# YannDubs/disentangling-vae

Measured on NVIDIA H100. Metric: images/sec, higher is better.
Workload: dtype f32

## Files before the change

disentangling-vae_b200/csrc/dv_conv_tc.cu:

```cuda
#include "dv_common.cuh"
#include "dv_ptx.cuh"

namespace dv {
namespace tc {

using namespace ptx;

constexpr int kATile = 128 * 128;
constexpr int kBTap = 64 * 128;
constexpr int kBBytes = kTaps * kBTap;
constexpr int kConsumers = 8;
constexpr int kThreads = (kConsumers + 1) * 32;
constexpr int kSmemMax = 232448;

__device__ __forceinline__ void consumers_sync() { asm volatile("bar.sync 1, %0;" ::"n"(kConsumers * 32) : "memory"); }

__device__ __forceinline__ void fold_tap(float (&tot)[16], float (&acc)[16]) {
  fence_regs(acc);
#pragma unroll
  for (int i = 0; i < 16; ++i) tot[i] += acc[i];
}

__device__ __forceinline__ void product(float (&acc)[16], float (&acc_prev)[16], float (&corr)[16], float (&tot)[16],
                                        uint32_t (&ah)[16], uint32_t (&al)[16], uint32_t a_base, int p0, int p1,
                                        uint32_t keep0, uint32_t keep1, int t, uint32_t tap_base, int corr_accumulate) {
#pragma unroll
  for (int ks = 0; ks < 4; ++ks) {
    wgmma_wait<3>();
    if (ks == 3) fold_tap(tot, acc_prev);
    split_tf32(lds32(a_base + swz128(p0, 8 * ks + t)) & keep0, ah[4 * ks + 0], al[4 * ks + 0]);
    split_tf32(lds32(a_base + swz128(p1, 8 * ks + t)) & keep1, ah[4 * ks + 1], al[4 * ks + 1]);
    split_tf32(lds32(a_base + swz128(p0, 8 * ks + t + 4)) & keep0, ah[4 * ks + 2], al[4 * ks + 2]);
    split_tf32(lds32(a_base + swz128(p1, 8 * ks + t + 4)) & keep1, ah[4 * ks + 3], al[4 * ks + 3]);
    fence_regs(acc);
    fence_regs(corr);
    wgmma_fence();
    const uint64_t w_hi = wgmma_desc_k128(tap_base + 32 * ks), w_lo = wgmma_desc_k128(tap_base + 32 * 128 + 32 * ks);
    wgmma_m64n32k8_rs(acc, ah + 4 * ks, w_hi, ks);
    wgmma_m64n32k8_rs(corr, ah + 4 * ks, w_lo, ks | corr_accumulate);
    wgmma_m64n32k8_rs(corr, al + 4 * ks, w_hi, 1);
    wgmma_commit();
  }
}

struct DownGeom {
  int B, H, W;
  int rows_per_tile;
  int num_tiles;
  long long total_px;
};
constexpr int kDownStages = 5;
struct DownBarriers {
  uint64_t raw_full[kDownStages], raw_empty[kDownStages];
  uint64_t b_full;
  float bias[32];
  float csum[kConsumers][32];
};
constexpr int kDownSmem = kBBytes + kDownStages * kATile + 1024 + 2048;
static_assert(sizeof(DownBarriers) <= 2048, "barrier block too large");
static_assert(kDownSmem <= kSmemMax, "smem");

__global__ void __launch_bounds__(kThreads, 1)
conv_down32_mma_kernel(const __grid_constant__ CUtensorMap tmap_a, const __grid_constant__ CUtensorMap tmap_b,
                       const float* __restrict__ bias, const float* __restrict__ mask, float* __restrict__ lo,
                       DownGeom g, int act, float* __restrict__ colsum_part,
                       const uint32_t* __restrict__ mask_bits, uint32_t* __restrict__ bits_out) {
  extern __shared__ uint8_t smem_raw[];
  uint8_t* smem = align1024(smem_raw);
  uint8_t* Bs = smem;
  uint8_t* Raw = smem + kBBytes;
  DownBarriers* bars = reinterpret_cast<DownBarriers*>(Raw + kDownStages * kATile);
  const int warp = threadIdx.x >> 5, lane = threadIdx.x & 31;
  if (threadIdx.x == 0) {
    for (int s = 0; s < kDownStages; ++s) { mbar_init(&bars->raw_full[s], 1); mbar_init(&bars->raw_empty[s], kConsumers); }
    mbar_init(&bars->b_full, 1);
    fence_mbar_init();
  }
  if (threadIdx.x < 32) bars->bias[threadIdx.x] = bias ? bias[threadIdx.x] : 0.f;
  __syncthreads();

  if (warp == kConsumers) {
    if (lane != 0) return;
    prefetch_tmap(&tmap_a); prefetch_tmap(&tmap_b);
    mbar_arrive_expect_tx(&bars->b_full, kBBytes);
    for (int tap = 0; tap < kTaps; ++tap) tma_load_2d(Bs + tap * kBTap, &tmap_b, &bars->b_full, 0, tap * 64);
    int stage = 0; uint32_t phase = 0;
    for (int tile = blockIdx.x; tile < g.num_tiles; tile += gridDim.x) {
      const int r0 = tile * g.rows_per_tile;
      const int b0 = r0 / g.H, i0 = r0 % g.H;
      if (tile + (int)gridDim.x < g.num_tiles) {
        const int rn = (tile + gridDim.x) * g.rows_per_tile;
        const int bn = rn / g.H, in_ = rn % g.H;
        for (int t4 = 0; t4 < 4; ++t4) tma_prefetch_4d(&tmap_a, 0, (t4 & 1), 2 * in_ + (t4 >> 1), bn);
      }
      for (int tap = 0; tap < kTaps; ++tap) {
        const int kh = tap >> 2, kw = tap & 3;
        mbar_wait(&bars->raw_empty[stage], phase ^ 1);
        mbar_arrive_expect_tx(&bars->raw_full[stage], kATile);
        tma_load_4d(Raw + stage * kATile, &tmap_a, &bars->raw_full[stage], 0, kw - 1, 2 * i0 - 1 + kh, b0);
        if (++stage == kDownStages) { stage = 0; phase ^= 1; }
      }
    }
    return;
  }

  const int gq = lane >> 2, t = lane & 3;
  const int r0 = warp * 16 + gq;
  const uint32_t bs = smem_u32(Bs), raw0 = smem_u32(Raw);
  float csum[4][2] = {};
  mbar_wait(&bars->b_full, 0);
  int stage = 0; uint32_t phase = 0;
  uint32_t ah[16], al[16];
  auto tap_product = [&](float (&acc)[16], float (&acc_prev)[16], float (&corr)[16], float (&tot)[16], int tap) {
    mbar_wait(&bars->raw_full[stage], phase);
    product(acc, acc_prev, corr, tot, ah, al, raw0 + stage * kATile, r0, r0 + 8, ~0u, ~0u, t, bs + tap * kBTap, tap);
    __syncwarp();
    if (lane == 0) mbar_arrive(&bars->raw_empty[stage]);
    if (++stage == kDownStages) { stage = 0; phase ^= 1; }
  };
  for (int tile = blockIdx.x; tile < g.num_tiles; tile += gridDim.x) {
    float tot[16] = {}, corr[16], acc[2][16];
#pragma unroll
    for (int i = 0; i < 16; ++i) acc[1][i] = 0.f;
#pragma unroll 1
    for (int tap = 0; tap < kTaps; tap += 2) {
      tap_product(acc[0], acc[1], corr, tot, tap);
      tap_product(acc[1], acc[0], corr, tot, tap + 1);
    }
    wgmma_wait<0>();
    fold_tap(tot, acc[1]);
    fence_regs(corr);
#pragma unroll
    for (int h = 0; h < 2; ++h) {
      const long long p = (long long)tile * 128 + r0 + 8 * h;
      const bool valid = p < g.total_px;
      uint32_t mb = 0xffffffffu;
      if (mask_bits && valid) mb = __ldg(mask_bits + p);
      const float* mk = (mask && !mask_bits && valid) ? mask + p * 32 : nullptr;
      uint32_t ob = 0u;
#pragma unroll
      for (int nt = 0; nt < 4; ++nt) {
        const int c = nt * 8 + 2 * t;
        float v[2];
#pragma unroll
        for (int e = 0; e < 2; ++e) {
          float x = (tot[4 * nt + 2 * h + e] + corr[4 * nt + 2 * h + e]) + bars->bias[c + e];
          if (act == DV_ACT_RELU) x = fmaxf(x, 0.f);
          v[e] = ((mb >> (c + e)) & 1u) ? x : 0.f;
        }
        if (mk) {
          const float2 m2 = __ldg(reinterpret_cast<const float2*>(mk + c));
          v[0] = m2.x > 0.f ? v[0] : 0.f; v[1] = m2.y > 0.f ? v[1] : 0.f;
        }
        if (valid) *reinterpret_cast<float2*>(lo + p * 32 + c) = make_float2(v[0], v[1]);
        else v[0] = v[1] = 0.f;
        ob |= (v[0] > 0.f ? 1u : 0u) << c | (v[1] > 0.f ? 1u : 0u) << (c + 1);
        csum[nt][0] += v[0]; csum[nt][1] += v[1];
      }
      ob |= __shfl_xor_sync(0xffffffffu, ob, 1);
      ob |= __shfl_xor_sync(0xffffffffu, ob, 2);
      if (bits_out && valid && t == 0) bits_out[p] = ob;
    }
  }
  if (colsum_part) {
#pragma unroll
    for (int nt = 0; nt < 4; ++nt)
#pragma unroll
      for (int e = 0; e < 2; ++e) {
        float s = csum[nt][e];
        s += __shfl_xor_sync(0xffffffffu, s, 4);
        s += __shfl_xor_sync(0xffffffffu, s, 8);
        s += __shfl_xor_sync(0xffffffffu, s, 16);
        if (gq == 0) bars->csum[warp][nt * 8 + 2 * t + e] = s;
      }
    consumers_sync();
    if (warp == 0) {
      float s = 0.f;
      for (int w = 0; w < kConsumers; ++w) s += bars->csum[w][lane];
      colsum_part[blockIdx.x * 32 + lane] = s;
    }
  }
}

constexpr int kWtSlots = kConsumers;
struct WtBarriers {
  uint64_t raw_full[kWtSlots], raw_empty[kWtSlots];
  uint64_t l_full[2], l_empty[2];
  float lsum[kConsumers][32];
};
constexpr int kWtTotFloats = 2 * 32 * 32;
constexpr int kWtSmem = kWtSlots * kATile + 2 * kATile + 2048 + kConsumers * kWtTotFloats * 4 + 1024;
static_assert(sizeof(WtBarriers) <= 2048, "barrier block too large");
static_assert(kWtSmem <= kSmemMax, "smem");

struct WtGeom {
  int B, H, W, rows_per_tile, num_tiles, tiles_per_cta;
};

__global__ void __launch_bounds__(kThreads, 1)
conv_wgrad32_mma_kernel(const __grid_constant__ CUtensorMap tmap_hi, const __grid_constant__ CUtensorMap tmap_lo,
                        float* __restrict__ ws, WtGeom g) {
  extern __shared__ uint8_t smem_raw[];
  uint8_t* smem = align1024(smem_raw);
  uint8_t* Raw = smem;
  uint8_t* Ls = smem + kWtSlots * kATile;
  WtBarriers* bars = reinterpret_cast<WtBarriers*>(Ls + 2 * kATile);
  const int warp = threadIdx.x >> 5, lane = threadIdx.x & 31;
  float* tot = reinterpret_cast<float*>(Ls + 2 * kATile + 2048) + warp * kWtTotFloats + lane;
  const int t_begin = blockIdx.x * g.tiles_per_cta;
  const int t_end = min(g.num_tiles, t_begin + g.tiles_per_cta);

  if (threadIdx.x == 0) {
    for (int s = 0; s < kWtSlots; ++s) { mbar_init(&bars->raw_full[s], 1); mbar_init(&bars->raw_empty[s], 1); }
    for (int s = 0; s < 2; ++s) { mbar_init(&bars->l_full[s], 1); mbar_init(&bars->l_empty[s], kConsumers); }
    fence_mbar_init();
  }
  __syncthreads();

  if (warp == kConsumers) {
    if (lane != 0) return;
    prefetch_tmap(&tmap_hi); prefetch_tmap(&tmap_lo);
    uint32_t tseq = 0;
    for (int tile = t_begin; tile < t_end; ++tile, ++tseq) {
      const int r0 = tile * g.rows_per_tile;
      const int b0 = r0 / g.H, i0 = r0 % g.H;
      if (tile + 1 < t_end) {
        const int rn = (tile + 1) * g.rows_per_tile;
        const int bn = rn / g.H, in_ = rn % g.H;
        for (int t4 = 0; t4 < 4; ++t4) tma_prefetch_4d(&tmap_hi, 0, (t4 & 1), 2 * in_ + (t4 >> 1), bn);
        tma_prefetch_4d(&tmap_lo, 0, 0, in_, bn);
      }
      const int lb = tseq & 1;
      mbar_wait(&bars->l_empty[lb], ((tseq >> 1) & 1u) ^ 1u);
      mbar_arrive_expect_tx(&bars->l_full[lb], kATile);
      tma_load_4d(Ls + lb * kATile, &tmap_lo, &bars->l_full[lb], 0, 0, i0, b0);
      for (int tap = 0; tap < kTaps; ++tap) {
        const int kh = tap >> 2, kw = tap & 3, slot = tap & 7;
        const uint32_t use = tseq * 2 + (tap >> 3);
        mbar_wait(&bars->raw_empty[slot], (use & 1u) ^ 1u);
        mbar_arrive_expect_tx(&bars->raw_full[slot], kATile);
        tma_load_4d(Raw + slot * kATile, &tmap_hi, &bars->raw_full[slot], 0, kw - 1, 2 * i0 - 1 + kh, b0);
      }
    }
    return;
  }

  const int gq = lane >> 2, t = lane & 3;
  const uint32_t slot_base = smem_u32(Raw) + warp * kATile, l0 = smem_u32(Ls);
  for (int k = 0; k < 64; ++k) tot[k * 32] = 0.f;
  float lsum = 0.f;
  uint32_t tseq = 0;
  for (int tile = t_begin; tile < t_end; ++tile, ++tseq) {
    const int lb = tseq & 1;
    mbar_wait(&bars->l_full[lb], (tseq >> 1) & 1u);
    const uint32_t l_base = l0 + lb * kATile;
#pragma unroll 4
    for (int r = 0; r < 16; ++r) lsum += __uint_as_float(lds32(l_base + swz128(warp * 16 + r, lane)));
#pragma unroll 1
    for (int j = 0; j < 2; ++j) {
      const uint32_t use = tseq * 2 + j;
      mbar_wait(&bars->raw_full[warp], use & 1u);
      float mn[2][4][4] = {}, cr[2][4][4] = {};
#pragma unroll 1
      for (int ks = 0; ks < 16; ++ks) {
        const int px0 = 8 * ks + 2 * t, px1 = px0 + 1;
        uint32_t ah[2][4], al[2][4], bh[4][2], bl[4][2];
#pragma unroll
        for (int mt = 0; mt < 2; ++mt) {
          const int c = mt * 16 + gq;
          uint32_t a[4];
          a[0] = lds32(slot_base + swz128(px0, c));
          a[1] = lds32(slot_base + swz128(px0, c + 8));
          a[2] = lds32(slot_base + swz128(px1, c));
          a[3] = lds32(slot_base + swz128(px1, c + 8));
#pragma unroll
          for (int e = 0; e < 4; ++e) split_tf32(a[e], ah[mt][e], al[mt][e]);
        }
#pragma unroll
        for (int nt = 0; nt < 4; ++nt) {
          const int cl = nt * 8 + gq;
          split_tf32(lds32(l_base + swz128(px0, cl)), bh[nt][0], bl[nt][0]);
          split_tf32(lds32(l_base + swz128(px1, cl)), bh[nt][1], bl[nt][1]);
        }
#pragma unroll
        for (int mt = 0; mt < 2; ++mt)
#pragma unroll
          for (int nt = 0; nt < 4; ++nt) mma_3xtf32(mn[mt][nt], cr[mt][nt], ah[mt], al[mt], bh[nt], bl[nt]);
      }
      __syncwarp();
      if (lane == 0) mbar_arrive(&bars->raw_empty[warp]);
#pragma unroll
      for (int mt = 0; mt < 2; ++mt)
#pragma unroll
        for (int nt = 0; nt < 4; ++nt)
#pragma unroll
          for (int e = 0; e < 4; ++e) tot[(j * 32 + (mt * 4 + nt) * 4 + e) * 32] += mn[mt][nt][e] + cr[mt][nt][e];
    }
    __syncwarp();
    if (lane == 0) mbar_arrive(&bars->l_empty[lb]);
  }

  float* out = ws + (long long)blockIdx.x * (kTaps * 32 + 1) * kLoCh;
#pragma unroll
  for (int j = 0; j < 2; ++j) {
    const int tap = warp + 8 * j;
#pragma unroll
    for (int mt = 0; mt < 2; ++mt)
#pragma unroll
      for (int nt = 0; nt < 4; ++nt)
#pragma unroll
        for (int h = 0; h < 2; ++h) {
          const int c = mt * 16 + gq + 8 * h, cl = nt * 8 + 2 * t;
          *reinterpret_cast<float2*>(out + (tap * 32 + c) * kLoCh + cl) =
              make_float2(tot[(j * 32 + (mt * 4 + nt) * 4 + 2 * h) * 32], tot[(j * 32 + (mt * 4 + nt) * 4 + 2 * h + 1) * 32]);
        }
  }
  bars->lsum[warp][lane] = lsum;
  consumers_sync();
  if (warp == 0) {
    float s = 0.f;
    for (int w = 0; w < kConsumers; ++w) s += bars->lsum[w][lane];
    out[(kTaps * 32) * kLoCh + lane] = s;
  }
}

constexpr int kHaloStageBytes = 26 * 1024;
constexpr int kHaloStages = 3;
struct HaloGeom {
  int B, H, W, TR, TB, tiles_per_img, num_tiles, valid_rows, box_px, box_bytes;
};
struct HaloBarriers {
  uint64_t raw_full[kHaloStages], raw_empty[kHaloStages];
  uint64_t b_full;
  float bias[32];
};
constexpr int kHaloSmem = kBBytes + kHaloStages * kHaloStageBytes + 1024 + 1024;
static_assert(sizeof(HaloBarriers) <= 1024, "barrier block too large");
static_assert(kHaloSmem <= kSmemMax, "smem");

__global__ void __launch_bounds__(kThreads, 1)
conv_up_halo_mma_kernel(const __grid_constant__ CUtensorMap tmap_a, const __grid_constant__ CUtensorMap tmap_b,
                        const float* __restrict__ bias, const float* __restrict__ mask, float* __restrict__ hi_out,
                        HaloGeom g, int act, const uint32_t* __restrict__ mask_bits, uint32_t* __restrict__ bits_out) {
  extern __shared__ uint8_t smem_raw[];
  uint8_t* smem = align1024(smem_raw);
  uint8_t* Bs = smem;
  uint8_t* Raw = smem + kBBytes;
  HaloBarriers* bars = reinterpret_cast<HaloBarriers*>(Raw + kHaloStages * kHaloStageBytes);
  const int warp = threadIdx.x >> 5, lane = threadIdx.x & 31;

  if (threadIdx.x == 0) {
    for (int s = 0; s < kHaloStages; ++s) { mbar_init(&bars->raw_full[s], 1); mbar_init(&bars->raw_empty[s], kConsumers); }
    mbar_init(&bars->b_full, 1);
    fence_mbar_init();
  }
  if (threadIdx.x < 32) bars->bias[threadIdx.x] = bias ? bias[threadIdx.x] : 0.f;
  __syncthreads();

  if (warp == kConsumers) {
    if (lane != 0) return;
    prefetch_tmap(&tmap_a); prefetch_tmap(&tmap_b);
    mbar_arrive_expect_tx(&bars->b_full, kBBytes);
    for (int tap = 0; tap < kTaps; ++tap) tma_load_2d(Bs + tap * kBTap, &tmap_b, &bars->b_full, 0, tap * 64);
    uint32_t t_seq = 0;
    for (int tile = blockIdx.x; tile < g.num_tiles; tile += gridDim.x, ++t_seq) {
      const int stage = t_seq % kHaloStages;
      int b0, i0;
      if (g.TB > 1) { b0 = tile * g.TB; i0 = 0; } else { b0 = tile / g.tiles_per_img; i0 = (tile % g.tiles_per_img) * g.TR; }
      mbar_wait(&bars->raw_empty[stage], ((t_seq / kHaloStages) & 1u) ^ 1u);
      mbar_arrive_expect_tx(&bars->raw_full[stage], g.box_bytes);
      tma_load_4d(Raw + stage * kHaloStageBytes, &tmap_a, &bars->raw_full[stage], 0, 0, i0 - 1, b0);
    }
    return;
  }

  const int gq = lane >> 2, t = lane & 3;
  const int HH = 2 * g.H, WW = 2 * g.W;
  const uint32_t bs = smem_u32(Bs), raw0 = smem_u32(Raw);
  int rj[2], src0[2];
  bool row_ok[2];
#pragma unroll
  for (int h = 0; h < 2; ++h) {
    const int row = warp * 16 + gq + 8 * h;
    const int rt = row / g.W, rtb = rt / g.TR;
    rj[h] = row - rt * g.W;
    src0[h] = min((rtb * (g.TR + 2) + (rt - rtb * g.TR) + 1) * g.W + rj[h], g.box_px - 1);
    row_ok[h] = row < g.valid_rows;
  }
  uint32_t ah[16], al[16];
  mbar_wait(&bars->b_full, 0);
  uint32_t t_seq = 0;
  for (int tile = blockIdx.x; tile < g.num_tiles; tile += gridDim.x, ++t_seq) {
    const int stage = t_seq % kHaloStages;
    const uint32_t a_base = raw0 + stage * kHaloStageBytes;
    mbar_wait(&bars->raw_full[stage], (t_seq / kHaloStages) & 1u);
    int b0, i0;
    if (g.TB > 1) { b0 = tile * g.TB; i0 = 0; } else { b0 = tile / g.tiles_per_img; i0 = (tile % g.tiles_per_img) * g.TR; }
#pragma unroll 1
    for (int pidx = 0; pidx < 4; ++pidx) {
      const int ph = pidx >> 1, pw = pidx & 1;
      float tot[16] = {}, corr[16], acc[2][16];
#pragma unroll
      for (int i = 0; i < 16; ++i) acc[1][i] = 0.f;
#pragma unroll
      for (int q = 0; q < 4; ++q) {
        const int di = ph - 1 + (q >> 1), dj = pw - 1 + (q & 1);
        const uint32_t b_base = bs + ((3 - ph - 2 * (q >> 1)) * 4 + 3 - pw - 2 * (q & 1)) * kBTap;
        int p[2];
        uint32_t keep[2];
#pragma unroll
        for (int h = 0; h < 2; ++h) {
          const bool ok = row_ok[h] && (unsigned)(rj[h] + dj) < (unsigned)g.W;
          p[h] = ok ? src0[h] + di * g.W + dj : src0[h];
          keep[h] = ok ? 0xffffffffu : 0u;
        }
        product(acc[q & 1], acc[(q + 1) & 1], corr, tot, ah, al, a_base, p[0], p[1], keep[0], keep[1], t, b_base, q);
      }
      wgmma_wait<0>();
      fold_tap(tot, acc[1]);
      fence_regs(corr);
#pragma unroll
      for (int h = 0; h < 2; ++h) {
        const int r = warp * 16 + gq + 8 * h, tr = r / g.W;
        const int tb = tr / g.TR, rr = tr - tb * g.TR;
        const int b = b0 + tb, i = i0 + rr, j = r - tr * g.W;
        const bool valid = r < g.valid_rows && b < g.B && i < g.H;
        const long long opix = valid ? ((long long)(b * HH + 2 * i + ph) * WW + 2 * j + pw) : 0;
        uint32_t mb = 0xffffffffu;
        if (mask_bits && valid) mb = __ldg(mask_bits + opix);
        const float* mk = (mask && !mask_bits && valid) ? mask + opix * 32 : nullptr;
        uint32_t ob = 0u;
#pragma unroll
        for (int nt = 0; nt < 4; ++nt) {
          const int c = nt * 8 + 2 * t;
          float v[2];
#pragma unroll
          for (int e = 0; e < 2; ++e) {
            float x = (tot[4 * nt + 2 * h + e] + corr[4 * nt + 2 * h + e]) + bars->bias[c + e];
            if (act == DV_ACT_RELU) x = fmaxf(x, 0.f);
            v[e] = ((mb >> (c + e)) & 1u) ? x : 0.f;
          }
          if (mk) {
            const float2 m2 = __ldg(reinterpret_cast<const float2*>(mk + c));
            v[0] = m2.x > 0.f ? v[0] : 0.f; v[1] = m2.y > 0.f ? v[1] : 0.f;
          }
          if (valid) *reinterpret_cast<float2*>(hi_out + opix * 32 + c) = make_float2(v[0], v[1]);
          ob |= (v[0] > 0.f ? 1u : 0u) << c | (v[1] > 0.f ? 1u : 0u) << (c + 1);
        }
        ob |= __shfl_xor_sync(0xffffffffu, ob, 1);
        ob |= __shfl_xor_sync(0xffffffffu, ob, 2);
        if (bits_out && valid && t == 0) bits_out[opix] = ob;
      }
    }
    __syncwarp();
    if (lane == 0) mbar_arrive(&bars->raw_empty[stage]);
  }
}

constexpr int kPackMultiMax = 8;
struct ConvPackTable {
  const float* w[kPackMultiMax];
  float* wp[kPackMultiMax];
  int CH[kPackMultiMax];
};
__global__ void conv_pack_multi_kernel(ConvPackTable tab) {
  const float* __restrict__ w = tab.w[blockIdx.y];
  float* __restrict__ wp = tab.wp[blockIdx.y];
  const int CH = tab.CH[blockIdx.y];
  const int n = kLoCh * CH * kTaps;
  for (int idx = blockIdx.x * blockDim.x + threadIdx.x; idx < n; idx += gridDim.x * blockDim.x) {
    const int tap = idx % kTaps, c = (idx / kTaps) % CH, cl = idx / (kTaps * CH);
    const float v = w[idx];
    if (CH != 32) {
      wp[(tap * CH + c) * kLoCh + cl] = v;
      wp[n + (tap * CH + c) * kLoCh + cl] = v;
      continue;
    }
    float* wd = wp;
    float* wu = wp + kTaps * 64 * 32;
    const float hi = tf32_round(v);
    const float lo = tf32_round(v - hi);
    wd[(tap * 64 + cl) * 32 + c] = hi;
    wd[(tap * 64 + 32 + cl) * 32 + c] = lo;
    wu[(tap * 64 + c) * 32 + cl] = hi;
    wu[(tap * 64 + 32 + c) * 32 + cl] = lo;
  }
}

static bool make_act_tmap(CUtensorMap* m, const float* base, int B, int HH, int WW, int bw, int bh, int bb, int stride) {
  EncodeTiledFn enc = get_encode();
  if (!enc) return false;
  cuuint64_t gdim[4] = {32, (cuuint64_t)WW, (cuuint64_t)HH, (cuuint64_t)B};
  cuuint64_t gstr[3] = {128, (cuuint64_t)WW * 128, (cuuint64_t)HH * WW * 128};
  cuuint32_t box[4] = {32, (cuuint32_t)bw, (cuuint32_t)bh, (cuuint32_t)bb};
  cuuint32_t estr[4] = {1, (cuuint32_t)stride, (cuuint32_t)stride, 1};
  return enc(m, CU_TENSOR_MAP_DATA_TYPE_FLOAT32, 4, const_cast<float*>(base), gdim, gstr, box, estr,
             CU_TENSOR_MAP_INTERLEAVE_NONE, CU_TENSOR_MAP_SWIZZLE_128B, CU_TENSOR_MAP_L2_PROMOTION_L2_128B,
             CU_TENSOR_MAP_FLOAT_OOB_FILL_NONE) == CUDA_SUCCESS;
}
static bool make_w_tmap(CUtensorMap* m, const float* base) {
  EncodeTiledFn enc = get_encode();
  if (!enc) return false;
  cuuint64_t gdim[2] = {32, (cuuint64_t)kTaps * 64};
  cuuint64_t gstr[1] = {128};
  cuuint32_t box[2] = {32, 64};
  cuuint32_t estr[2] = {1, 1};
  return enc(m, CU_TENSOR_MAP_DATA_TYPE_FLOAT32, 2, const_cast<float*>(base), gdim, gstr, box, estr,
             CU_TENSOR_MAP_INTERLEAVE_NONE, CU_TENSOR_MAP_SWIZZLE_128B, CU_TENSOR_MAP_L2_PROMOTION_L2_128B,
             CU_TENSOR_MAP_FLOAT_OOB_FILL_NONE) == CUDA_SUCCESS;
}

int pack_multi(int n, const float* const* w, float* const* wp, const int* CH, cudaStream_t st) {
  for (int base = 0; base < n; base += kPackMultiMax) {
    ConvPackTable tab = {};
    const int m = n - base < kPackMultiMax ? n - base : kPackMultiMax;
    for (int i = 0; i < m; ++i) { tab.w[i] = w[base + i]; tab.wp[i] = wp[base + i]; tab.CH[i] = CH[base + i]; }
    conv_pack_multi_kernel<<<dim3(16, m), 256, 0, st>>>(tab);
    const int rc = check_launch();
    if (rc != DV_OK) return rc;
  }
  return DV_OK;
}

int conv_down32_tc(const float* hi, const float* wd_packed, const float* bias, const float* mask, float* lo,
                   int B, int H, int W, int act, cudaStream_t st, float* colsum_part, int* nparts,
                   const uint32_t* mask_bits, uint32_t* bits_out) {
  if (nparts) *nparts = 0;
  if (W > 128 || 128 % W != 0) return DV_ERR_BAD_SHAPE;
  DownGeom g = {};
  g.B = B; g.H = H; g.W = W;
  g.rows_per_tile = 128 / W;
  const int TR = g.rows_per_tile < H ? g.rows_per_tile : H;
  if (H % TR != 0 || g.rows_per_tile % TR != 0) return DV_ERR_BAD_SHAPE;
  const int TB = g.rows_per_tile / TR;
  g.total_px = (long long)B * H * W;
  g.num_tiles = (int)((g.total_px + 127) / 128);
  CUtensorMap ta, tb;
  if (!make_act_tmap(&ta, hi, B, 2 * H, 2 * W, 2 * W, 2 * TR, TB, 2)) return DV_ERR_CUDA;
  if (!make_w_tmap(&tb, wd_packed)) return DV_ERR_CUDA;
  static bool attr = false;
  const int rc = set_max_dynamic_smem(conv_down32_mma_kernel, kDownSmem, &attr);
  if (rc != DV_OK) return rc;
  const int grid = g.num_tiles < kNumSMs ? g.num_tiles : kNumSMs;
  conv_down32_mma_kernel<<<grid, kThreads, kDownSmem, st>>>(ta, tb, bias, mask, lo, g, act, colsum_part, mask_bits, bits_out);
  if (nparts && colsum_part) *nparts = grid;
  return check_launch();
}

int wgrad_splits(int B, int H, int W) {
  const int num_tiles = (int)(((long long)B * H * W + 127) / 128);
  const int grid = num_tiles < kNumSMs ? num_tiles : kNumSMs;
  const int tiles_per_cta = (num_tiles + grid - 1) / grid;
  return (num_tiles + tiles_per_cta - 1) / tiles_per_cta;
}

int conv_wgrad32_tc(const float* lo, const float* hi, float* ws, int B, int H, int W, cudaStream_t st) {
  if (W > 128 || 128 % W != 0) return DV_ERR_BAD_SHAPE;
  WtGeom g = {};
  g.B = B; g.H = H; g.W = W;
  g.rows_per_tile = 128 / W;
  const int TR = g.rows_per_tile < H ? g.rows_per_tile : H;
  if (H % TR != 0 || g.rows_per_tile % TR != 0) return DV_ERR_BAD_SHAPE;
  const int TB = g.rows_per_tile / TR;
  g.num_tiles = (int)(((long long)B * H * W + 127) / 128);
  const int grid = wgrad_splits(B, H, W);
  g.tiles_per_cta = (g.num_tiles + grid - 1) / grid;
  CUtensorMap thi, tlo;
  if (!make_act_tmap(&thi, hi, B, 2 * H, 2 * W, 2 * W, 2 * TR, TB, 2)) return DV_ERR_CUDA;
  if (!make_act_tmap(&tlo, lo, B, H, W, W, TR, TB, 1)) return DV_ERR_CUDA;
  static bool attr = false;
  const int rc = set_max_dynamic_smem(conv_wgrad32_mma_kernel, kWtSmem, &attr);
  if (rc != DV_OK) return rc;
  conv_wgrad32_mma_kernel<<<grid, kThreads, kWtSmem, st>>>(thi, tlo, ws, g);
  return check_launch();
}

int conv_up_halo(const float* lo, const float* wu, const float* bias, const float* mask, float* hi,
                 int B, int H, int W, int act, cudaStream_t st, const uint32_t* mask_bits, uint32_t* bits_out) {
  HaloGeom g = {};
  g.B = B; g.H = H; g.W = W;
  if (W > 32 || 128 % W != 0) return DV_ERR_BAD_SHAPE;
  const int rpt = 128 / W;
  if (rpt >= H) {
    g.TR = H;
    g.TB = rpt / H < 1 ? 1 : rpt / H;
    while (g.TB > 1 && g.TB * (H + 2) * W * 128 > kHaloStageBytes) --g.TB;
    g.tiles_per_img = 1;
    g.num_tiles = (B + g.TB - 1) / g.TB;
  } else {
    g.TR = rpt; g.TB = 1;
    g.tiles_per_img = (H + rpt - 1) / rpt;
    g.num_tiles = B * g.tiles_per_img;
  }
  g.valid_rows = g.TB * g.TR * W;
  g.box_px = g.TB * (g.TR + 2) * W;
  g.box_bytes = g.box_px * 128;
  if (g.box_bytes > kHaloStageBytes) return DV_ERR_BAD_SHAPE;
  CUtensorMap ta, tb;
  if (!make_act_tmap(&ta, lo, g.B, g.H, g.W, g.W, g.TR + 2, g.TB, 1)) return DV_ERR_CUDA;
  if (!make_w_tmap(&tb, wu)) return DV_ERR_CUDA;
  static bool attr = false;
  const int rc = set_max_dynamic_smem(conv_up_halo_mma_kernel, kHaloSmem, &attr);
  if (rc != DV_OK) return rc;
  const int grid = g.num_tiles < kNumSMs ? g.num_tiles : kNumSMs;
  conv_up_halo_mma_kernel<<<grid, kThreads, kHaloSmem, st>>>(ta, tb, bias, mask, hi, g, act, mask_bits, bits_out);
  return check_launch();
}

}
}
```

disentangling-vae_b200/csrc/dv_ptx.cuh:

```cuda
#pragma once
#include <cuda.h>
#include <cuda_runtime.h>
#include <stdint.h>

namespace dv {
namespace ptx {

__device__ __forceinline__ uint32_t smem_u32(const void* p) {
  return static_cast<uint32_t>(__cvta_generic_to_shared(p));
}

__device__ __forceinline__ void mbar_init(uint64_t* bar, uint32_t count) {
  asm volatile("mbarrier.init.shared::cta.b64 [%0], %1;" ::"r"(smem_u32(bar)), "r"(count));
}
__device__ __forceinline__ void fence_mbar_init() {
  asm volatile("fence.mbarrier_init.release.cluster;" ::: "memory");
}
__device__ __forceinline__ void mbar_arrive(uint64_t* bar) {
  asm volatile("mbarrier.arrive.shared::cta.b64 _, [%0];" ::"r"(smem_u32(bar)) : "memory");
}
__device__ __forceinline__ void mbar_arrive_expect_tx(uint64_t* bar, uint32_t bytes) {
  asm volatile("mbarrier.arrive.expect_tx.shared::cta.b64 _, [%0], %1;" ::"r"(smem_u32(bar)), "r"(bytes) : "memory");
}
__device__ __forceinline__ void mbar_wait(uint64_t* bar, uint32_t parity) {
  const uint32_t addr = smem_u32(bar);
  uint32_t done = 0;
  for (uint32_t spin = 0; !done; ++spin) {
    asm volatile(
        "{\n\t.reg .pred p;\n\t"
        "mbarrier.try_wait.parity.shared::cta.b64 p, [%1], %2;\n\t"
        "selp.u32 %0, 1, 0, p;\n\t}"
        : "=r"(done)
        : "r"(addr), "r"(parity)
        : "memory");
    if (spin > (1u << 24)) __trap();
  }
}

__device__ __forceinline__ uint32_t lds32(uint32_t smem_addr) {
  uint32_t v;
  asm volatile("ld.shared.u32 %0, [%1];" : "=r"(v) : "r"(smem_addr) : "memory");
  return v;
}

__device__ __forceinline__ uint32_t swz128(int r, int c) {
  return (uint32_t)(r * 128 + ((((c >> 2) ^ (r & 7)) << 4) | ((c & 3) << 2)));
}

__device__ __forceinline__ void prefetch_tmap(const CUtensorMap* m) {
  asm volatile("prefetch.tensormap [%0];" ::"l"(reinterpret_cast<uint64_t>(m)) : "memory");
}
__device__ __forceinline__ void tma_load_4d(void* smem_dst, const CUtensorMap* m, uint64_t* bar, int c0, int c1, int c2, int c3) {
  asm volatile(
      "cp.async.bulk.tensor.4d.shared::cluster.global.mbarrier::complete_tx::bytes [%0], [%1, {%3, %4, %5, %6}], [%2];"
      ::"r"(smem_u32(smem_dst)), "l"(reinterpret_cast<uint64_t>(m)), "r"(smem_u32(bar)), "r"(c0), "r"(c1), "r"(c2), "r"(c3)
      : "memory");
}
__device__ __forceinline__ void tma_load_2d(void* smem_dst, const CUtensorMap* m, uint64_t* bar, int c0, int c1) {
  asm volatile(
      "cp.async.bulk.tensor.2d.shared::cluster.global.mbarrier::complete_tx::bytes [%0], [%1, {%3, %4}], [%2];"
      ::"r"(smem_u32(smem_dst)), "l"(reinterpret_cast<uint64_t>(m)), "r"(smem_u32(bar)), "r"(c0), "r"(c1)
      : "memory");
}
__device__ __forceinline__ void tma_prefetch_4d(const CUtensorMap* m, int c0, int c1, int c2, int c3) {
  asm volatile("cp.async.bulk.prefetch.tensor.4d.L2.global.tile [%0, {%1, %2, %3, %4}];"
               ::"l"(reinterpret_cast<uint64_t>(m)), "r"(c0), "r"(c1), "r"(c2), "r"(c3) : "memory");
}

typedef CUresult (*EncodeTiledFn)(CUtensorMap*, CUtensorMapDataType, cuuint32_t, void*, const cuuint64_t*, const cuuint64_t*,
                                  const cuuint32_t*, const cuuint32_t*, CUtensorMapInterleave, CUtensorMapSwizzle,
                                  CUtensorMapL2promotion, CUtensorMapFloatOOBfill);
inline EncodeTiledFn get_encode() {
  static const EncodeTiledFn fn = [] {
    void* p = nullptr;
    cudaDriverEntryPointQueryResult qres;
    const bool ok = cudaGetDriverEntryPoint("cuTensorMapEncodeTiled", &p, cudaEnableDefault, &qres) == cudaSuccess &&
                    qres == cudaDriverEntryPointSuccess;
    return ok ? reinterpret_cast<EncodeTiledFn>(p) : nullptr;
  }();
  return fn;
}

__device__ __forceinline__ float tf32_round(float x) {
  return __uint_as_float((__float_as_uint(x) + 0x1000u) & 0xFFFFE000u);
}
__device__ __forceinline__ void split_tf32(uint32_t x, uint32_t& hi, uint32_t& lo) {
  const float h = tf32_round(__uint_as_float(x));
  hi = __float_as_uint(h);
  lo = __float_as_uint(tf32_round(__uint_as_float(x) - h));
}

__device__ __forceinline__ void mma_tf32(float (&d)[4], const uint32_t (&a)[4], const uint32_t (&b)[2]) {
  asm volatile(
      "mma.sync.aligned.m16n8k8.row.col.f32.tf32.tf32.f32 {%0, %1, %2, %3}, {%4, %5, %6, %7}, {%8, %9}, {%0, %1, %2, %3};"
      : "+f"(d[0]), "+f"(d[1]), "+f"(d[2]), "+f"(d[3])
      : "r"(a[0]), "r"(a[1]), "r"(a[2]), "r"(a[3]), "r"(b[0]), "r"(b[1]));
}

__device__ __forceinline__ void mma_3xtf32(float (&main)[4], float (&corr)[4], const uint32_t (&a_hi)[4],
                                           const uint32_t (&a_lo)[4], const uint32_t (&b_hi)[2], const uint32_t (&b_lo)[2]) {
  mma_tf32(main, a_hi, b_hi);
  mma_tf32(corr, a_hi, b_lo);
  mma_tf32(corr, a_lo, b_hi);
}

__device__ __forceinline__ uint64_t wgmma_desc_k128(uint32_t smem_addr) {
  return (uint64_t)((smem_addr & 0x3FFFFu) >> 4) | ((uint64_t)1 << 16) | ((uint64_t)(1024 >> 4) << 32) | ((uint64_t)1 << 62);
}
__device__ __forceinline__ void wgmma_fence() { asm volatile("wgmma.fence.sync.aligned;" ::: "memory"); }
__device__ __forceinline__ void wgmma_commit() { asm volatile("wgmma.commit_group.sync.aligned;" ::: "memory"); }
template <int N>
__device__ __forceinline__ void wgmma_wait() { asm volatile("wgmma.wait_group.sync.aligned %0;" ::"n"(N) : "memory"); }
template <int N>
__device__ __forceinline__ void fence_regs(float (&r)[N]) {
#pragma unroll
  for (int i = 0; i < N; ++i) asm volatile("" : "+f"(r[i])::"memory");
}

__device__ __forceinline__ void wgmma_m64n32k8_rs(float (&d)[16], const uint32_t* a, uint64_t b_desc, int accumulate) {
  asm volatile(
      "{\n\t.reg .pred p;\n\tsetp.ne.b32 p, %21, 0;\n\t"
      "wgmma.mma_async.sync.aligned.m64n32k8.f32.tf32.tf32 "
      "{%0, %1, %2, %3, %4, %5, %6, %7, %8, %9, %10, %11, %12, %13, %14, %15}, "
      "{%16, %17, %18, %19}, %20, p, 1, 1;\n\t}"
      : "+f"(d[0]), "+f"(d[1]), "+f"(d[2]), "+f"(d[3]), "+f"(d[4]), "+f"(d[5]), "+f"(d[6]), "+f"(d[7]),
        "+f"(d[8]), "+f"(d[9]), "+f"(d[10]), "+f"(d[11]), "+f"(d[12]), "+f"(d[13]), "+f"(d[14]), "+f"(d[15])
      : "r"(a[0]), "r"(a[1]), "r"(a[2]), "r"(a[3]), "l"(b_desc), "r"(accumulate));
}

}
}
```

Before: 444,000.

## Port weight-gradient conv kernel from mma.sync to warpgroup wgmma

Rewrites the 32-channel weight-gradient kernel to use Hopper wgmma m64n32k8 with register A operands and shared-memory B descriptors instead of per-warp mma.sync 3xTF32. The low-resolution activations are now pre-split once per tile into hi/lo TF32 planes in shared memory, written in swizzled layout and made visible with a proxy fence. Each tap slot is consumed by two warps through a 7-slot ring instead of one slot per warp, and the L buffer drops from double to single buffering. This aims to cut the repeated B-operand splitting and raise tensor-core throughput. In exchange it adds consumer-wide barriers per tile and removes the overlap that double buffering gave.

```diff
diff --git a/disentangling-vae_b200/csrc/dv_conv_tc.cu b/disentangling-vae_b200/csrc/dv_conv_tc.cu
--- a/disentangling-vae_b200/csrc/dv_conv_tc.cu
+++ b/disentangling-vae_b200/csrc/dv_conv_tc.cu
@@ -182,14 +182,15 @@
   }
 }
 
-constexpr int kWtSlots = kConsumers;
+constexpr int kWtSlots = 7;
+constexpr int kWtPlane = 32 * 128 * 4;
 struct WtBarriers {
   uint64_t raw_full[kWtSlots], raw_empty[kWtSlots];
-  uint64_t l_full[2], l_empty[2];
+  uint64_t l_full, l_empty;
   float lsum[kConsumers][32];
 };
-constexpr int kWtTotFloats = 2 * 32 * 32;
-constexpr int kWtSmem = kWtSlots * kATile + 2 * kATile + 2048 + kConsumers * kWtTotFloats * 4 + 1024;
+constexpr int kWtTotFloats = 4 * 16 * 32;
+constexpr int kWtSmem = kWtSlots * kATile + kATile + 2 * kWtPlane + 2048 + kConsumers * kWtTotFloats * 4 + 1024;
 static_assert(sizeof(WtBarriers) <= 2048, "barrier block too large");
 static_assert(kWtSmem <= kSmemMax, "smem");
 
@@ -198,21 +199,22 @@
 };
 
 __global__ void __launch_bounds__(kThreads, 1)
-conv_wgrad32_mma_kernel(const __grid_constant__ CUtensorMap tmap_hi, const __grid_constant__ CUtensorMap tmap_lo,
-                        float* __restrict__ ws, WtGeom g) {
+conv_wgrad32_wgmma_kernel(const __grid_constant__ CUtensorMap tmap_hi, const __grid_constant__ CUtensorMap tmap_lo,
+                          float* __restrict__ ws, WtGeom g) {
   extern __shared__ uint8_t smem_raw[];
   uint8_t* smem = align1024(smem_raw);
   uint8_t* Raw = smem;
   uint8_t* Ls = smem + kWtSlots * kATile;
-  WtBarriers* bars = reinterpret_cast<WtBarriers*>(Ls + 2 * kATile);
+  uint8_t* Planes = Ls + kATile;
+  WtBarriers* bars = reinterpret_cast<WtBarriers*>(Planes + 2 * kWtPlane);
   const int warp = threadIdx.x >> 5, lane = threadIdx.x & 31;
-  float* tot = reinterpret_cast<float*>(Ls + 2 * kATile + 2048) + warp * kWtTotFloats + lane;
+  float* tot = reinterpret_cast<float*>(Planes + 2 * kWtPlane + 2048) + warp * kWtTotFloats + lane;
   const int t_begin = blockIdx.x * g.tiles_per_cta;
   const int t_end = min(g.num_tiles, t_begin + g.tiles_per_cta);
 
   if (threadIdx.x == 0) {
-    for (int s = 0; s < kWtSlots; ++s) { mbar_init(&bars->raw_full[s], 1); mbar_init(&bars->raw_empty[s], 1); }
-    for (int s = 0; s < 2; ++s) { mbar_init(&bars->l_full[s], 1); mbar_init(&bars->l_empty[s], kConsumers); }
+    for (int s = 0; s < kWtSlots; ++s) { mbar_init(&bars->raw_full[s], 1); mbar_init(&bars->raw_empty[s], 2); }
+    mbar_init(&bars->l_full, 1); mbar_init(&bars->l_empty, kConsumers);
     fence_mbar_init();
   }
   __syncthreads();
@@ -220,7 +222,7 @@
   if (warp == kConsumers) {
     if (lane != 0) return;
     prefetch_tmap(&tmap_hi); prefetch_tmap(&tmap_lo);
-    uint32_t tseq = 0;
+    int slot = 0; uint32_t phase = 0, tseq = 0;
     for (int tile = t_begin; tile < t_end; ++tile, ++tseq) {
       const int r0 = tile * g.rows_per_tile;
       const int b0 = r0 / g.H, i0 = r0 % g.H;
@@ -230,90 +232,99 @@
         for (int t4 = 0; t4 < 4; ++t4) tma_prefetch_4d(&tmap_hi, 0, (t4 & 1), 2 * in_ + (t4 >> 1), bn);
         tma_prefetch_4d(&tmap_lo, 0, 0, in_, bn);
       }
-      const int lb = tseq & 1;
-      mbar_wait(&bars->l_empty[lb], ((tseq >> 1) & 1u) ^ 1u);
-      mbar_arrive_expect_tx(&bars->l_full[lb], kATile);
-      tma_load_4d(Ls + lb * kATile, &tmap_lo, &bars->l_full[lb], 0, 0, i0, b0);
+      mbar_wait(&bars->l_empty, (tseq & 1u) ^ 1u);
+      mbar_arrive_expect_tx(&bars->l_full, kATile);
+      tma_load_4d(Ls, &tmap_lo, &bars->l_full, 0, 0, i0, b0);
       for (int tap = 0; tap < kTaps; ++tap) {
-        const int kh = tap >> 2, kw = tap & 3, slot = tap & 7;
-        const uint32_t use = tseq * 2 + (tap >> 3);
-        mbar_wait(&bars->raw_empty[slot], (use & 1u) ^ 1u);
+        const int kh = tap >> 2, kw = tap & 3;
+        mbar_wait(&bars->raw_empty[slot], phase ^ 1);
         mbar_arrive_expect_tx(&bars->raw_full[slot], kATile);
         tma_load_4d(Raw + slot * kATile, &tmap_hi, &bars->raw_full[slot], 0, kw - 1, 2 * i0 - 1 + kh, b0);
+        if (++slot == kWtSlots) { slot = 0; phase ^= 1; }
       }
     }
     return;
   }
 
-  const int gq = lane >> 2, t = lane & 3;
-  const uint32_t slot_base = smem_u32(Raw) + warp * kATile, l0 = smem_u32(Ls);
+  const int gq = lane >> 2, t = lane & 3, wg = warp >> 2, wq = warp & 3;
+  const uint32_t raw0 = smem_u32(Raw), l_base = smem_u32(Ls), planes = smem_u32(Planes);
+  const int c0 = (wq & 1) * 16 + gq;
+  const uint32_t a_off[4] = {swz128(2 * t, c0), swz128(2 * t, c0 + 8), swz128(2 * t + 1, c0), swz128(2 * t + 1, c0 + 8)};
   for (int k = 0; k < 64; ++k) tot[k * 32] = 0.f;
   float lsum = 0.f;
   uint32_t tseq = 0;
   for (int tile = t_begin; tile < t_end; ++tile, ++tseq) {
-    const int lb = tseq & 1;
-    mbar_wait(&bars->l_full[lb], (tseq >> 1) & 1u);
-    const uint32_t l_base = l0 + lb * kATile;
-#pragma unroll 4
-    for (int r = 0; r < 16; ++r) lsum += __uint_as_float(lds32(l_base + swz128(warp * 16 + r, lane)));
+    mbar_wait(&bars->l_full, tseq & 1u);
+    consumers_sync();
+    {
+      uint32_t v[16];
+#pragma unroll
+      for (int r = 0; r < 16; ++r) v[r] = lds32(l_base + swz128(warp * 16 + r, lane));
+#pragma unroll
+      for (int r = 0; r < 16; ++r) lsum += __uint_as_float(v[r]);
+      __syncwarp();
+      if (lane == 0) mbar_arrive(&bars->l_empty);
+#pragma unroll
+      for (int h = 0; h < 2; ++h)
+#pragma unroll
+        for (int par = 0; par < 2; ++par) {
+          const int ks = 2 * warp + h;
+          uint32_t ph[4], pl[4];
+#pragma unroll
+          for (int q = 0; q < 4; ++q) split_tf32(v[8 * h + 2 * q + par], ph[q], pl[q]);
+          const uint32_t dst = planes + (ks >> 2) * 4096 + swz128(lane, 8 * (ks & 3) + 4 * par);
+          sts128(dst, ph);
+          sts128(dst + kWtPlane, pl);
+        }
+    }
+    fence_proxy_async();
+    consumers_sync();
 #pragma unroll 1
-    for (int j = 0; j < 2; ++j) {
-      const uint32_t use = tseq * 2 + j;
-      mbar_wait(&bars->raw_full[warp], use & 1u);
-      float mn[2][4][4] = {}, cr[2][4][4] = {};
+    for (int j = 0; j < 4; ++j) {
+      const uint32_t n = tseq * kTaps + 4 * j + 2 * wg + (wq >> 1);
+      const uint32_t slot = n % kWtSlots;
+      mbar_wait(&bars->raw_full[slot], (n / kWtSlots) & 1u);
+      const uint32_t a_base = raw0 + slot * kATile;
+      float acc[16], corr[16];
+      uint32_t ah[16], al[16];
 #pragma unroll 1
-      for (int ks = 0; ks < 16; ++ks) {
-        const int px0 = 8 * ks + 2 * t, px1 = px0 + 1;
-        uint32_t ah[2][4], al[2][4], bh[4][2], bl[4][2];
-#pragma unroll
-        for (int mt = 0; mt < 2; ++mt) {
-          const int c = mt * 16 + gq;
-          uint32_t a[4];
-          a[0] = lds32(slot_base + swz128(px0, c));
-          a[1] = lds32(slot_base + swz128(px0, c + 8));
-          a[2] = lds32(slot_base + swz128(px1, c));
-          a[3] = lds32(slot_base + swz128(px1, c + 8));
-#pragma unroll
-          for (int e = 0; e < 4; ++e) split_tf32(a[e], ah[mt][e], al[mt][e]);
+      for (int kb = 0; kb < 4; ++kb) {
+#pragma unroll
+        for (int k4 = 0; k4 < 4; ++k4) {
+          const int ks = 4 * kb + k4;
+          wgmma_wait<3>();
+#pragma unroll
+          for (int e = 0; e < 4; ++e) split_tf32(lds32(a_base + 1024 * ks + a_off[e]), ah[4 * k4 + e], al[4 * k4 + e]);
+          fence_regs(acc);
+          fence_regs(corr);
+          wgmma_fence();
+          const uint64_t b_hi = wgmma_desc_k128(planes + kb * 4096 + 32 * k4), b_lo = wgmma_desc_k128(planes + kWtPlane + kb * 4096 + 32 * k4);
+          wgmma_m64n32k8_rs(acc, ah + 4 * k4, b_hi, ks);
+          wgmma_m64n32k8_rs(corr, ah + 4 * k4, b_lo, ks);
+          wgmma_m64n32k8_rs(corr, al + 4 * k4, b_hi, 1);
+          wgmma_commit();
         }
-#pragma unroll
-        for (int nt = 0; nt < 4; ++nt) {
-          const int cl = nt * 8 + gq;
-          split_tf32(lds32(l_base + swz128(px0, cl)), bh[nt][0], bl[nt][0]);
-          split_tf32(lds32(l_base + swz128(px1, cl)), bh[nt][1], bl[nt][1]);
-        }
-#pragma unroll
-        for (int mt = 0; mt < 2; ++mt)
-#pragma unroll
-          for (int nt = 0; nt < 4; ++nt) mma_3xtf32(mn[mt][nt], cr[mt][nt], ah[mt], al[mt], bh[nt], bl[nt]);
       }
       __syncwarp();
-      if (lane == 0) mbar_arrive(&bars->raw_empty[warp]);
-#pragma unroll
-      for (int mt = 0; mt < 2; ++mt)
-#pragma unroll
-        for (int nt = 0; nt < 4; ++nt)
-#pragma unroll
-          for (int e = 0; e < 4; ++e) tot[(j * 32 + (mt * 4 + nt) * 4 + e) * 32] += mn[mt][nt][e] + cr[mt][nt][e];
-    }
-    __syncwarp();
-    if (lane == 0) mbar_arrive(&bars->l_empty[lb]);
+      if (lane == 0) mbar_arrive(&bars->raw_empty[slot]);
+      wgmma_wait<0>();
+      fence_regs(acc);
+      fence_regs(corr);
+#pragma unroll
+      for (int i = 0; i < 16; ++i) tot[(j * 16 + i) * 32] += acc[i] + corr[i];
+    }
   }
 
   float* out = ws + (long long)blockIdx.x * (kTaps * 32 + 1) * kLoCh;
 #pragma unroll
-  for (int j = 0; j < 2; ++j) {
-    const int tap = warp + 8 * j;
-#pragma unroll
-    for (int mt = 0; mt < 2; ++mt)
-#pragma unroll
-      for (int nt = 0; nt < 4; ++nt)
-#pragma unroll
-        for (int h = 0; h < 2; ++h) {
-          const int c = mt * 16 + gq + 8 * h, cl = nt * 8 + 2 * t;
-          *reinterpret_cast<float2*>(out + (tap * 32 + c) * kLoCh + cl) =
-              make_float2(tot[(j * 32 + (mt * 4 + nt) * 4 + 2 * h) * 32], tot[(j * 32 + (mt * 4 + nt) * 4 + 2 * h + 1) * 32]);
-        }
+  for (int j = 0; j < 4; ++j) {
+    const int tap = 4 * j + 2 * wg + (wq >> 1);
+#pragma unroll
+    for (int nt = 0; nt < 4; ++nt)
+#pragma unroll
+      for (int h = 0; h < 2; ++h)
+        *reinterpret_cast<float2*>(out + (tap * 32 + c0 + 8 * h) * kLoCh + nt * 8 + 2 * t) =
+            make_float2(tot[(j * 16 + 4 * nt + 2 * h) * 32], tot[(j * 16 + 4 * nt + 2 * h + 1) * 32]);
   }
   bars->lsum[warp][lane] = lsum;
   consumers_sync();
@@ -569,9 +580,9 @@
   if (!make_act_tmap(&thi, hi, B, 2 * H, 2 * W, 2 * W, 2 * TR, TB, 2)) return DV_ERR_CUDA;
   if (!make_act_tmap(&tlo, lo, B, H, W, W, TR, TB, 1)) return DV_ERR_CUDA;
   static bool attr = false;
-  const int rc = set_max_dynamic_smem(conv_wgrad32_mma_kernel, kWtSmem, &attr);
+  const int rc = set_max_dynamic_smem(conv_wgrad32_wgmma_kernel, kWtSmem, &attr);
   if (rc != DV_OK) return rc;
-  conv_wgrad32_mma_kernel<<<grid, kThreads, kWtSmem, st>>>(thi, tlo, ws, g);
+  conv_wgrad32_wgmma_kernel<<<grid, kThreads, kWtSmem, st>>>(thi, tlo, ws, g);
   return check_launch();
 }
 
diff --git a/disentangling-vae_b200/csrc/dv_ptx.cuh b/disentangling-vae_b200/csrc/dv_ptx.cuh
--- a/disentangling-vae_b200/csrc/dv_ptx.cuh
+++ b/disentangling-vae_b200/csrc/dv_ptx.cuh
@@ -42,6 +42,11 @@
   asm volatile("ld.shared.u32 %0, [%1];" : "=r"(v) : "r"(smem_addr) : "memory");
   return v;
 }
+
+__device__ __forceinline__ void sts128(uint32_t smem_addr, const uint32_t (&v)[4]) {
+  asm volatile("st.shared.v4.u32 [%0], {%1, %2, %3, %4};" ::"r"(smem_addr), "r"(v[0]), "r"(v[1]), "r"(v[2]), "r"(v[3]) : "memory");
+}
+__device__ __forceinline__ void fence_proxy_async() { asm volatile("fence.proxy.async.shared::cta;" ::: "memory"); }
 
 __device__ __forceinline__ uint32_t swz128(int r, int c) {
   return (uint32_t)(r * 128 + ((((c >> 2) ^ (r & 7)) << 4) | ((c & 3) << 2)));
```

After: 460,900 (median of 6 runs). 1.04x the previous value.
